# UbiquityRobotics/fiducials

Measured on AMD Instinct MI355X. Metric: frames/sec @1920x1080 20-marker (aruco detect + pose hot path), higher is better.
Workload: dtype u8

## Files before the change

fiducials_amd/csrc/fid_api.hip:

```cpp
#include "fid_kernels.hip"

#include <math.h>
#include <stdio.h>
#include <stdlib.h>
#include <string.h>

#include <new>
#include <string>
#include <vector>

namespace {

enum { ST_GRAY = 0, ST_THRESH, ST_STARTS, ST_PROBE, ST_WALK, ST_APPROX, ST_SORT, ST_NEAR, ST_RESOLVE, ST_IDENT, ST_FILTER, ST_SUBPIX, ST_POSE, ST_SEEDWALK,
       ST_SEEDLESS, ST_COUNT };
const char *const kStageNames[ST_COUNT] = {"to_gray", "threshold", "find_starts", "walk_probe", "walk_full", "approx", "sort_cands",
                                           "near", "resolve", "identify", "filter_markers", "subpix", "pose", "seed_walk", "seedless_chain"};

constexpr int TX = 128, TY = 32, NT = 256;
constexpr int THRW_NT = 512, THRW_WT = 16;
static_assert(THRW_NT * THRW_WT >= 8191, "k_threshold_wide: a row per workgroup");

}

struct fid_ctx {
    int device = 0;
    hipStream_t stream = nullptr;
    enum { MAX_SUB = 8 };
    hipStream_t sub_stream[MAX_SUB] = {};
    int sub_prio[MAX_SUB] = {};
    hipStream_t aux_stream[MAX_SUB] = {};
    hipStream_t idx_stream = nullptr;
    hipEvent_t aux_fork[MAX_SUB] = {}, aux_join[MAX_SUB] = {}, aux_idx[MAX_SUB] = {};
    hipEvent_t sub_done[MAX_SUB] = {}, fork_ev = nullptr;
    hipStream_t copy_stream = nullptr;
    hipEvent_t in_ready[MAX_SUB] = {};
    bool host_feed = false;
    struct Pending {
        const uint8_t *d_src;
        int F, W, H, stride;
        long long fstride;
        fid_encoding enc;
    } pend = {};
    bool in_flight = false;
    hipEvent_t tail_ev = nullptr, wait_ev = nullptr;
    hipEvent_t wait_copy_ev = nullptr;
    bool fed_from_host = false;
    int chain_at = 0;
    bool chained = false;
    hipEvent_t walk_done[MAX_SUB] = {}, fs_done[MAX_SUB] = {}, front_done[MAX_SUB] = {};
    int pieces = 0;
    bool piece_chain = false;
    bool from_host_call = false;
    int fs_barrier = 0;
    int stagger = 0;
    int resolve_lds_kb = 64;
    int walk2_div = 6;
    int probe_refill0 = 0;
    int probe_refill = 4;
    hipEvent_t sub_ev[MAX_SUB][20] = {};
    int sub_frames = 0;
    fid_params params;
    fid_limits lim;
    DevParams P;
    std::vector<uint8_t> dict_host;
    int dict_ms = 0, dict_maxc = 0, dict_n = 0;
    uint8_t *d_in = nullptr;
    size_t d_in_bytes = 0;
    uint8_t *d_gray = nullptr;
    uint32_t *d_masks = nullptr;
    size_t masks_bytes = 0;
    int masks_W = 0, masks_H = 0, masks_S = 0;
    uint2 *d_starts = nullptr, *d_surv1 = nullptr, *d_surv = nullptr;
    uint32_t *d_pool = nullptr;
    DevSegC *d_segs = nullptr;
    DevPend *d_pend = nullptr;
    uint2 *d_seedq = nullptr;
    unsigned long long *d_seedhash = nullptr;
    int seed_hash_cap = 0, seed_gen = 0;
    uint4 *d_wres = nullptr, *d_cinfo = nullptr;
    uint32_t *d_cbase = nullptr, *d_dense = nullptr;
    uint4 *d_recs = nullptr;
    int thr_xcd = 1;
    int thr_nw = 3, thr_split = 0, thr_rows = 0;
    bool whole_border_walk = false;
    int sw_blocks = 0;
    int tail_grid = 4096;
    int filter_lds = 256;
    int light_x = 1;
    long long fallbacks = 0;
    int max_chunks = 0;
    int walk_blocks = 0;
    int walk_blocks_cap = 0;
    int copy_blocks = 0;
    int resolve_serial = 0;
    int resolve_reg_max = 64;
    int seed_shift = 0;
    uint4 *d_contours = nullptr;
    uint32_t *d_ckpts = nullptr;
    size_t ckpts_elems = 0;
    DevCand *d_cands = nullptr, *d_sorted = nullptr, *d_filtered = nullptr;
    float4 *d_cmeta = nullptr;
    uint32_t *d_near = nullptr;
    DevIdent *d_ident = nullptr;
    uint8_t *d_bits = nullptr;
    int bits_cap = 0;
    fid_marker *d_pre = nullptr, *d_markers = nullptr, *d_filter_scratch = nullptr;
    int *d_accsrc = nullptr, *d_mksrc = nullptr;
    fid_pose_out *d_poses = nullptr;
    DevCounts *d_counts = nullptr;
    DevGlobal *d_global = nullptr;
    unsigned *d_worklist = nullptr, *d_nwork = nullptr;
    uint8_t *d_dict = nullptr;
    float *d_subpix_mask = nullptr;
    uint8_t *d_probe_tables = nullptr;
    double *d_lens = nullptr;
    fid_marker *d_pose_in = nullptr;
    int *d_pose_n = nullptr;
    int pose_cap = 0;
    uint8_t *d_res = nullptr, *h_res = nullptr;
    size_t res_clear_bytes = 0, res_markers_end = 0, res_poses_end = 0, res_poses_off = 0;
    bool blocking = false;
    bool res_precleared = false;
    fid_marker *h_markers = nullptr;
    DevCounts *h_counts = nullptr;
    DevGlobal *h_global = nullptr;
    fid_pose_out *h_poses = nullptr;
    bool pose_cam_valid = false, pose_done = false;
    fid_camera pose_cam = {};
    double pose_len = 0.;
    int *d_map_ids = nullptr;
    double *d_map_obj = nullptr;
    int map_n = 0;
    fid_map_pose_out *d_mposes = nullptr, *h_mposes = nullptr;
    fid_marker *d_map_in = nullptr;
    int map_in_cap = 0;
    bool map_cam_valid = false, map_done = false;
    fid_camera map_cam = {};
    int last_frames = 0, last_W = 0, last_H = 0, last_nsub = 1;
    const uint8_t *last_gray = nullptr;
    long long last_gfstride = 0;
    bool profile = false;
    hipEvent_t ev[ST_COUNT + 1] = {};
    bool ev_valid[ST_COUNT + 1] = {};
    float stage_ms[ST_COUNT] = {};
    std::string last_error;
};

static void map_pose_launch(fid_ctx *c, hipStream_t st, const fid_marker *d_markers, const int *d_n, int n_stride_ints, int per_frame, int F,
                            const fid_camera &camera, fid_map_pose_out *d_out);

namespace {

#define HIPCHK(ctx, expr)                                                                         \
    do {                                                                                          \
        hipError_t e_ = (expr);                                                                   \
        if (e_ != hipSuccess) {                                                                   \
            (ctx)->last_error = std::string(#expr) + ": " + hipGetErrorString(e_);                \
            return e_ == hipErrorOutOfMemory ? FID_E_OUT_OF_MEMORY : FID_E_HIP;                   \
        }                                                                                         \
    } while (0)

template <typename T>
fid_status dalloc(fid_ctx *c, T **p, size_t count)
{
    HIPCHK(c, hipMalloc((void **)p, count * sizeof(T)));
    return FID_OK;
}

int roundup(int v, int m) { return (v + m - 1) / m * m; }

size_t results_bytes(int F, int MM)
{
    auto up = [](size_t v) { return (v + 255) & ~(size_t)255; };
    return up(sizeof(DevGlobal)) + up(sizeof(unsigned) * fid_ctx::MAX_SUB) + up(sizeof(DevCounts) * (size_t)F) + up(sizeof(fid_marker) * (size_t)F * MM) +
           up(sizeof(fid_pose_out) * (size_t)F * MM);
}
void layout_results(fid_ctx *c, int F)
{
    auto up = [](size_t v) { return (v + 255) & ~(size_t)255; };
// ... 306 lines not shown
        const fid_status rcs = ensure_streams(c, nsub, F);
        if (rcs != FID_OK) return rcs;
    }
    if (nsub > 1) HIPCHK(c, hipEventRecord(c->fork_ev, st0));
    bool tail_recorded = false;
    auto sub_phase = [&](int sb, int phase) -> fid_status {
        const int f0 = plan.f0[sb], Fs = plan.f0[sb + 1] - f0;
        hipStream_t st = nsub > 1 ? c->sub_stream[chainp ? (sb & 1) : sb] : st0;
        if (nsub > 1 && phase == 0) HIPCHK(c, hipStreamWaitEvent(st, c->fork_ev, 0));
        if (chainp && phase == 0 && sb > 0) HIPCHK(c, hipStreamWaitEvent(st, c->fs_done[sb - 1], 0));
        if (c->host_feed && phase == 0) HIPCHK(c, hipStreamWaitEvent(st, c->in_ready[sb], 0));
        if (nsub > 1 && phase == 0 && c->stagger > 0 && sb >= c->stagger) HIPCHK(c, hipStreamWaitEvent(st, c->walk_done[sb - c->stagger], 0));
        DevParams P = c->P;
        P.nframes = Fs;
        const size_t MC = (size_t)P.maxCands, MM = (size_t)P.maxMarkers;
        const uint8_t *g = gray + (long long)f0 * gfstride;
        uint32_t *masks = c->d_masks + (size_t)f0 * P.nscales * P.TR * P.TC * MT_ROWS;
        uint2 *starts = c->d_starts + (size_t)f0 * P.maxStarts, *surv1 = c->d_surv1 + (size_t)f0 * P.maxStarts,
              *surv = c->d_surv + (size_t)f0 * P.maxStarts;
        uint4 *contours = c->d_contours + (size_t)f0 * P.maxContours;
        uint32_t *tab = c->d_ckpts + (size_t)f0 * 2 * P.maxContours * chunk_tab_pitch(P);
        uint32_t *pool = c->d_pool + (size_t)f0 * P.maxChunks * CKW;
        DevCounts *counts = c->d_counts + f0;
        DevCand *cands = c->d_cands + f0 * MC, *sorted = c->d_sorted + f0 * MC, *filtered = c->d_filtered + f0 * MC;
        uint32_t *nearb = c->d_near + f0 * MC * (MC / 32);
        DevIdent *ident = c->d_ident + f0 * MC;
        fid_marker *pre = c->d_pre + f0 * MM, *markers = c->d_markers + f0 * MM;
        unsigned *worklist = c->d_worklist + f0 * MC, *nwork = c->d_nwork + sb;
        hipEvent_t *ev = c->sub_ev[sb];
        auto mark = [&](int idx) {
            if (c->profile) (void)hipEventRecord(ev[idx], st);
        };
        auto chain_point = [&](int pt) {
            if (sb == nsub - 1 && !tail_recorded && !c->blocking && c->chain_at <= pt) {
                (void)hipEventRecord(c->tail_ev, st);
                tail_recorded = true;
            }
        };
      if (phase == 0) {
        mark(0);
        if (to_gray && (int)enc <= FID_ENC_RGBA8)
            hipLaunchKernelGGL(k_to_gray, dim3(2048), dim3(256), 0, st, d_src + (long long)f0 * fstride, stride, fstride, (int)enc,
                               c->d_gray + (size_t)f0 * W * H, W, H, Fs);
        else if (to_gray)
            hipLaunchKernelGGL(k_raw_to_gray, dim3((W + 255) / 256, (H + 3) / 4, Fs), dim3(64, 4), 0, st, d_src + (long long)f0 * fstride, stride,
                               fstride, (int)enc, c->d_gray + (size_t)f0 * W * H, W, H);
        mark(ST_GRAY + 1);
        {
            bool node_table = P.nscales == 13;
            for (int i = 0; i < P.nscales && node_table; i++) node_table = P.win[i] == 3 + 4 * i;
            if (node_table) {
                const int cols = 64 * c->thr_nw, strips = (W + cols - 1) / cols;
                int RS = c->thr_rows;
                if (RS <= 0) {
                    int segs = (1536 + strips * Fs - 1) / (strips * Fs);
                    const int maxsegs = (H + 63) / 64;
                    segs = segs < 1 ? 1 : (segs > maxsegs ? maxsegs : segs);
                    RS = (H + segs - 1) / segs;
                }
                RS = (RS + 3) & ~3;
                dim3 grid(strips, (H + RS - 1) / RS, Fs);
                if (c->thr_nw == 5 && c->thr_split) launch_thr_stream<5, true>(grid, st, g, gfstride, masks, P, RS, c->thr_xcd);
                else if (c->thr_nw == 5) launch_thr_stream<5, false>(grid, st, g, gfstride, masks, P, RS, c->thr_xcd);
                else if (c->thr_split) launch_thr_stream<3, true>(grid, st, g, gfstride, masks, P, RS, c->thr_xcd);
                else launch_thr_stream<3, false>(grid, st, g, gfstride, masks, P, RS, c->thr_xcd);
            } else if (P.rmax > 40) {
                int bands = (512 + Fs - 1) / Fs;
                const int maxb = (H + 15) / 16;
                bands = bands < 1 ? 1 : (bands > maxb ? maxb : bands);
                const int BH = (H + bands - 1) / bands;
                const size_t lds = (size_t)(W + 1 + THRW_NT / 64) * sizeof(unsigned long long);
                fid_launch_log("k_threshold_wide", THRW_NT, lds);
                hipLaunchKernelGGL((k_threshold_wide<THRW_NT, THRW_WT>), dim3((H + BH - 1) / BH, 1, Fs), dim3(THRW_NT), lds, st, g, gfstride,
                                   masks, P, BH);
            } else {
                int R = P.rmax, RW = TX + 2 * R, RH = TY + 2 * R, PT = (RW + 1) | 1;
                size_t lds = (size_t)(RH + 1) * PT * sizeof(uint32_t);
                dim3 grid((W + TX - 1) / TX, (H + TY - 1) / TY, Fs);
                hipLaunchKernelGGL((k_threshold<TX, TY, NT>), grid, dim3(NT), lds, st, g, gfstride, masks, P);
            }
        }
        mark(ST_THRESH + 1);
      }
        long long k2blocks;
        {
            long long groups = (long long)P.nscales * P.TR * ((P.WW + 15) / 16);
            k2blocks = (groups + 7) / 8;
            if (k2blocks > 256) k2blocks = 256;
        }
      if (phase == 0) {
        if (!c->whole_border_walk) {
            hipLaunchKernelGGL(k_find_starts<true>, dim3((unsigned)k2blocks, Fs), dim3(256), 0, st, masks, starts, counts, c->d_global,
                               c->d_seedq + f0 * (size_t)P.maxContours, P);
            mark(ST_STARTS + 1);
            if (nsub > 1) HIPCHK(c, hipEventRecord(c->fs_done[sb], st));
            chain_point(0);
        }
        return FID_OK;
      }
        if (!c->whole_border_walk && nsub > 1 && c->fs_barrier && !chainp)
            for (int o = 0; o < nsub; o++)
                if (o != sb) HIPCHK(c, hipStreamWaitEvent(st, c->fs_done[o], 0));
        int wb = c->walk_blocks > 0 ? c->walk_blocks : (3072 / WALK_WAVES + Fs - 1) / Fs;
        const int wcap = c->walk_blocks_cap > 0 ? c->walk_blocks_cap : (Fs <= 2 ? 256 : 64);
        wb = wb < 2 ? 2 : (wb > wcap ? wcap : wb);
        const int gm = Fs >= 16 ? 1 : 16 / Fs;
        const int wb2 = wb > 1 ? wb / 2 : 1;
        const int cap1 = pts_cap_first(P);
        const size_t lds1 = k_approx_lds_bytes(cap1);
        const size_t lds2 = k_approx_lds_bytes(P.maxPerim + 1);
        if (c->whole_border_walk) {
            hipLaunchKernelGGL(k_find_starts<false>, dim3((unsigned)k2blocks, Fs), dim3(256), 0, st, masks, starts, counts, c->d_global,
                               (uint2 *)nullptr, P);
            mark(ST_STARTS + 1);
            hipLaunchKernelGGL((k_probe<PROBE0_STEPS, 0>), dim3(64 * gm, Fs), dim3(256), 0, st, masks, starts, surv1, counts, c->d_global, P);
            hipLaunchKernelGGL((k_probe<PROBE1_STEPS, 1>), dim3(16 * gm, Fs), dim3(256), 0, st, masks, surv1, surv, counts, c->d_global, P);
            mark(ST_PROBE + 1);
            hipLaunchKernelGGL(k_walk_full<0>, dim3(wb, Fs), dim3(64 * WALK_WAVES), 0, st, masks, surv, contours, tab, pool, (DevSegC *)nullptr,
                               (DevPend *)nullptr, counts, c->d_global, P);
            mark(ST_WALK + 1);
            fid_launch_log("k_approx", 64, (size_t)(lds1));
            hipLaunchKernelGGL(k_approx, dim3(128 * gm, Fs), dim3(64), lds1, st, contours, tab, pool, cands, counts, P, cap1, 0,
                               (const uint32_t *)nullptr, (const uint32_t *)nullptr);
            fid_launch_log("k_approx", 64, (size_t)(lds2));
            hipLaunchKernelGGL(k_approx, dim3(16 * gm, Fs), dim3(64), lds2, st, contours, tab, pool, cands, counts, P,
                               P.maxPerim + 1, 1, (const uint32_t *)nullptr, (const uint32_t *)nullptr);
            mark(ST_APPROX + 1);
        } else {
            const size_t MCn = (size_t)P.maxContours;
            DevSegC *segs = c->d_segs + f0 * MCn;
            DevPend *pend = c->d_pend + f0 * MCn;
            uint2 *seedq = c->d_seedq + f0 * MCn;
            unsigned long long *seedhash = c->d_seedhash + (size_t)f0 * P.seedHashCap;
            uint4 *wres = c->d_wres + f0 * MCn, *cinfo = c->d_cinfo + f0 * MCn;
            uint32_t *cbase = c->d_cbase + f0 * MCn;
            uint32_t *dense = c->d_dense + (size_t)f0 * P.maxChunks * (CK / 4);
            hipStream_t sa = c->aux_stream[chainp ? (sb & 1) : sb];
            HIPCHK(c, hipEventRecord(c->aux_fork[sb], st));
            HIPCHK(c, hipStreamWaitEvent(sa, c->aux_fork[sb], 0));
            int swb = c->sw_blocks > 0 ? c->sw_blocks : (1024 / SW_WAVES + Fs - 1) / Fs;
            swb = swb < 2 ? 2 : (swb > 4 * wcap ? 4 * wcap : swb);
            uint4 *recs = c->d_recs + 2 * f0 * MCn;
            const int cpb = c->copy_blocks > 0 ? c->copy_blocks : 256;
            if (c->profile) (void)hipEventRecord(ev[14], st);
            hipLaunchKernelGGL(k_seed_walk, dim3(swb, Fs), dim3(64 * SW_WAVES), 0, st, masks, seedq, tab, pool, segs, counts, c->d_global, P);
            if (c->profile) (void)hipEventRecord(ev[15], st);
            mark(ST_PROBE + 1);
            chain_point(1);
            if (c->profile) (void)hipEventRecord(ev[16], sa);
            hipStream_t si = (nsub == 1 && Fs <= 16 && c->idx_stream) ? c->idx_stream : sa;
            if (si != sa) HIPCHK(c, hipStreamWaitEvent(si, c->aux_fork[sb], 0));
            hipLaunchKernelGGL(k_seed_index, dim3(8 * gm, Fs), dim3(256), 0, si, seedq, seedhash, counts, P);
            HIPCHK(c, hipEventRecord(c->aux_idx[sb], si));
            if (c->probe_refill0 && gm == 1)
                hipLaunchKernelGGL((k_probe_refill<PROBE0_STEPS, 0>), dim3(c->probe_refill0, Fs), dim3(256), 0, sa, masks, starts, surv1, counts, c->d_global, P,
                                   (const uint4 *)c->d_probe_tables);
            else
                hipLaunchKernelGGL((k_probe_lut<PROBE0_STEPS, 0>), dim3(64 * gm, Fs), dim3(256), 0, sa, masks, starts, surv1, counts, c->d_global, P,
                                   (const uint4 *)c->d_probe_tables);
            if (c->probe_refill && gm == 1)
                hipLaunchKernelGGL((k_probe_refill<PROBE1_STEPS, 1>), dim3(c->probe_refill, Fs), dim3(256), 0, sa, masks, surv1, surv, counts, c->d_global, P,
                                   (const uint4 *)c->d_probe_tables);
            else
                hipLaunchKernelGGL((k_probe_lut<PROBE1_STEPS, 1>), dim3(16 * gm, Fs), dim3(256), 0, sa, masks, surv1, surv, counts, c->d_global, P,
                                   (const uint4 *)c->d_probe_tables);
            const int wb3 = c->walk2_div > 0 ? (wb / c->walk2_div > 0 ? wb / c->walk2_div : 1) : wb2;
            hipLaunchKernelGGL(k_walk_full<2>, dim3(wb3, Fs), dim3(64 * WALK_WAVES), 0, sa, masks, surv, wres, tab, pool, segs, pend, counts,
                               c->d_global, P);
            if (si != sa) HIPCHK(c, hipStreamWaitEvent(sa, c->aux_idx[sb], 0));
            hipLaunchKernelGGL(k_seg_cycles<0>, dim3(8 * gm, Fs), dim3(64), 0, sa, seedq, segs, pend, wres, contours, cinfo, cbase,
                               recs, counts, c->d_global, P, 1, 0);
            hipLaunchKernelGGL(k_seg_copy, dim3(cpb / 4 > 0 ? cpb / 4 : 1, Fs), dim3(256), 0, sa, recs, tab, pool, dense, counts, P, 1);
            fid_launch_log("k_approx", 64, (size_t)(lds1));
            hipLaunchKernelGGL(k_approx, dim3(32 * gm, Fs), dim3(64), lds1, sa, contours, tab, pool, cands, counts, P, cap1, 0,
                               dense, cbase, 2);
            fid_launch_log("k_approx", 64, (size_t)(lds2));
            hipLaunchKernelGGL(k_approx, dim3(8 * gm, Fs), dim3(64), lds2, sa, contours, tab, pool, cands, counts, P,
// ... 250 lines not shown
    memset(p, 0, sizeof(*p));
    p->adaptiveThreshConstant = 7;
    p->adaptiveThreshWinSizeMin = 3;
    p->adaptiveThreshWinSizeMax = 53;
    p->adaptiveThreshWinSizeStep = 4;
    p->cornerRefinementMethod = 1;
    p->cornerRefinementWinSize = 5;
    p->cornerRefinementMaxIterations = 30;
    p->cornerRefinementMinAccuracy = 0.01;
    p->errorCorrectionRate = 0.6;
    p->minCornerDistanceRate = 0.05;
    p->markerBorderBits = 1;
    p->minDistanceToBorder = 3;
    p->maxErroneousBitsInBorderRate = 0.04;
    p->minMarkerDistanceRate = 0.05;
    p->minMarkerPerimeterRate = 0.1;
    p->maxMarkerPerimeterRate = 4.0;
    p->minOtsuStdDev = 5.0;
    p->perspectiveRemoveIgnoredMarginPerCell = 0.13;
    p->perspectiveRemovePixelPerCell = 8;
    p->polygonalApproxAccuracyRate = 0.01;
}

void fid_default_limits(fid_limits *l)
{
    if (!l) return;
    memset(l, 0, sizeof(*l));
    l->max_width = 1920;
    l->max_height = 1080;
    l->max_batch = 1;
    l->max_starts_per_frame = 262144;
    l->max_contours_per_frame = 16384;
    l->max_candidates_per_frame = 2048;
    l->max_markers_per_frame = 256;
    l->max_points_per_frame = 4 * 1024 * 1024;
}

fid_status fid_create(const fid_params *params, const fid_dict *dict, const fid_limits *limits, int device, fid_ctx **out)
{
    if (!params || !dict || !out || !dict->bytes || dict->n_markers <= 0 || dict->marker_size < 3 || dict->marker_size > 7)
        return FID_E_INVALID_ARG;
    *out = nullptr;
    int ndev = 0;
    if (hipGetDeviceCount(&ndev) != hipSuccess || ndev <= 0) return FID_E_NO_DEVICE;
    if (device < 0 || device >= ndev) return FID_E_INVALID_ARG;
    fid_ctx *c = new (std::nothrow) fid_ctx();
    if (!c) return FID_E_OUT_OF_MEMORY;
    c->device = device;
    fid_limits L;
    fid_default_limits(&L);
    if (limits) {
        if (limits->max_width > 0) L.max_width = limits->max_width;
        if (limits->max_height > 0) L.max_height = limits->max_height;
        if (limits->max_batch > 0) L.max_batch = limits->max_batch;
        if (limits->max_starts_per_frame > 0) L.max_starts_per_frame = limits->max_starts_per_frame;
        if (limits->max_contours_per_frame > 0) L.max_contours_per_frame = limits->max_contours_per_frame;
        if (limits->max_candidates_per_frame > 0) L.max_candidates_per_frame = limits->max_candidates_per_frame;
        if (limits->max_markers_per_frame > 0) L.max_markers_per_frame = limits->max_markers_per_frame;
        if (limits->max_points_per_frame > 0) L.max_points_per_frame = limits->max_points_per_frame;
    }
    if (L.max_batch <= 4) {
        if (!limits || limits->max_contours_per_frame <= 0) L.max_contours_per_frame = 65536;
        if (!limits || limits->max_points_per_frame <= 0) L.max_points_per_frame = 16 * 1024 * 1024;
    } else if (L.max_batch <= 16) {
        if (!limits || limits->max_contours_per_frame <= 0) L.max_contours_per_frame = 32768;
        if (!limits || limits->max_points_per_frame <= 0) L.max_points_per_frame = 8 * 1024 * 1024;
    }
    L.max_candidates_per_frame = roundup(L.max_candidates_per_frame, 32);
    if (L.max_candidates_per_frame > 4096 || L.max_batch > 65535 || L.max_markers_per_frame > L.max_candidates_per_frame ||
        L.max_contours_per_frame > (1 << 20)) {
        delete c;
        return FID_E_INVALID_ARG;
    }
    c->lim = L;
    c->dict_ms = dict->marker_size;
    c->dict_maxc = dict->max_correction_bits;
    c->dict_n = dict->n_markers;
    size_t dbytes = (size_t)dict->n_markers * 4 * ((dict->marker_size * dict->marker_size + 7) / 8);
    c->dict_host.assign(dict->bytes, dict->bytes + dbytes);
    c->profile = getenv("FID_PROFILE") && atoi(getenv("FID_PROFILE")) != 0;
    if (getenv("FID_SUB_FRAMES")) c->sub_frames = atoi(getenv("FID_SUB_FRAMES"));
    if (getenv("FID_WALK_CAP")) c->walk_blocks_cap = atoi(getenv("FID_WALK_CAP"));
    if (getenv("FID_SEED_SHIFT")) c->seed_shift = atoi(getenv("FID_SEED_SHIFT"));
    if (getenv("FID_RESOLVE_SERIAL")) c->resolve_serial = atoi(getenv("FID_RESOLVE_SERIAL"));
    if (getenv("FID_RESOLVE_REG_MAX")) {
        const int v = atoi(getenv("FID_RESOLVE_REG_MAX"));
        c->resolve_reg_max = v < 0 ? 0 : (v > 64 ? 64 : v);
    }
    if (getenv("FID_COPY_BLOCKS")) c->copy_blocks = atoi(getenv("FID_COPY_BLOCKS"));
    if (getenv("FID_THR_NW")) c->thr_nw = atoi(getenv("FID_THR_NW")) == 3 ? 3 : 5;
    if (getenv("FID_THR_SPLIT")) c->thr_split = atoi(getenv("FID_THR_SPLIT")) != 0;
    if (getenv("FID_THR_ROWS")) c->thr_rows = atoi(getenv("FID_THR_ROWS"));
    if (getenv("FID_THR_XCD")) c->thr_xcd = atoi(getenv("FID_THR_XCD")) != 0;
    if (getenv("FID_WALK_BLOCKS")) c->walk_blocks = atoi(getenv("FID_WALK_BLOCKS")) > 0 ? atoi(getenv("FID_WALK_BLOCKS")) : c->walk_blocks;
    memset(&c->P, 0, sizeof(c->P));

    fid_status rc = FID_OK;
    auto fail = [&](fid_status s) {
        fid_destroy(c);
        return s;
    };
#define TRY(expr)                         \
    do {                                  \
        rc = (expr);                      \
        if (rc != FID_OK) return fail(rc); \
    } while (0)
#define TRYHIP(expr)                                   \
    do {                                               \
        hipError_t e_ = (expr);                        \
        if (e_ != hipSuccess) {                        \
            fprintf(stderr, "fid_create: %s: %s\n", #expr, hipGetErrorString(e_)); \
            return fail(e_ == hipErrorOutOfMemory ? FID_E_OUT_OF_MEMORY : FID_E_HIP); \
        }                                              \
    } while (0)
    TRYHIP(hipSetDevice(device));
    TRYHIP(hipStreamCreateWithFlags(&c->stream, hipStreamNonBlocking));
    for (int i = 0; i <= ST_COUNT; i++) TRYHIP(hipEventCreate(&c->ev[i]));
    TRYHIP(hipEventCreateWithFlags(&c->fork_ev, hipEventDisableTiming));
    TRYHIP(hipEventCreateWithFlags(&c->tail_ev, hipEventDisableTiming));
    int prio_lo = 0, prio_hi = 0;
    (void)hipDeviceGetStreamPriorityRange(&prio_lo, &prio_hi);
    const bool use_prio = getenv("FID_PRIO") && atoi(getenv("FID_PRIO"));
    for (int sb = 0; sb < fid_ctx::MAX_SUB; sb++) {
        int prio = use_prio ? prio_hi + sb : prio_lo;
        if (prio > prio_lo) prio = prio_lo;
        c->sub_prio[sb] = prio;
        TRYHIP(hipEventCreateWithFlags(&c->aux_fork[sb], hipEventDisableTiming));
        TRYHIP(hipEventCreateWithFlags(&c->aux_join[sb], hipEventDisableTiming));
        TRYHIP(hipEventCreateWithFlags(&c->sub_done[sb], hipEventDisableTiming));
        TRYHIP(hipEventCreateWithFlags(&c->walk_done[sb], hipEventDisableTiming));
        TRYHIP(hipEventCreateWithFlags(&c->in_ready[sb], hipEventDisableTiming));
        TRYHIP(hipEventCreateWithFlags(&c->fs_done[sb], hipEventDisableTiming));
        TRYHIP(hipEventCreateWithFlags(&c->front_done[sb], hipEventDisableTiming));
        TRYHIP(hipEventCreateWithFlags(&c->aux_idx[sb], hipEventDisableTiming));
        for (int i = 0; i < 20; i++) TRYHIP(hipEventCreate(&c->sub_ev[sb][i]));
    }
    const size_t F = L.max_batch, MC = L.max_candidates_per_frame, MM = L.max_markers_per_frame;
    TRY(dalloc(c, &c->d_subpix_mask, (size_t)(2 * SP_MAXWIN_MAX + 1) * (2 * SP_MAXWIN_MAX + 1)));
    TRY(dalloc(c, &c->d_probe_tables, (size_t)4096));
    hipLaunchKernelGGL(k_probe_tables, dim3(1), dim3(256), 0, nullptr, c->d_probe_tables);
    TRYHIP(hipGetLastError());
    TRYHIP(hipDeviceSynchronize());
    TRY(dalloc(c, &c->d_dict, dbytes));
    TRYHIP(hipMemcpy(c->d_dict, c->dict_host.data(), dbytes, hipMemcpyHostToDevice));
    rc = apply_params(c, params);
    if (rc != FID_OK) return fail(rc);
    TRY(dalloc(c, &c->d_gray, F * L.max_width * L.max_height));
    c->masks_bytes = masks_elems(c, L.max_width, L.max_height, (int)F) * sizeof(uint32_t);
    c->masks_bytes += (size_t)F * c->P.nscales * (L.max_height + 2) * 16 * sizeof(uint32_t);
    TRYHIP(hipMalloc((void **)&c->d_masks, c->masks_bytes));
    TRY(dalloc(c, &c->d_starts, F * L.max_starts_per_frame));
    TRY(dalloc(c, &c->d_surv1, F * L.max_starts_per_frame));
    TRY(dalloc(c, &c->d_surv, F * L.max_starts_per_frame));
    c->max_chunks = (L.max_points_per_frame + CK - 1) / CK;
    TRY(dalloc(c, &c->d_pool, F * (size_t)c->max_chunks * CKW));
    c->whole_border_walk = getenv("FID_TRACE") && !strcmp(getenv("FID_TRACE"), "legacy");
    if (getenv("FID_SW_BLOCKS")) c->sw_blocks = atoi(getenv("FID_SW_BLOCKS"));
    if (getenv("FID_STAGGER")) c->stagger = atoi(getenv("FID_STAGGER"));
    if (getenv("FID_PIECES")) c->pieces = atoi(getenv("FID_PIECES"));
    if (getenv("FID_FS_BARRIER")) c->fs_barrier = atoi(getenv("FID_FS_BARRIER"));
    if (getenv("FID_TAIL_GRID")) c->tail_grid = atoi(getenv("FID_TAIL_GRID"));
    if (getenv("FID_FILTER_LDS")) c->filter_lds = atoi(getenv("FID_FILTER_LDS")) > 0 ? atoi(getenv("FID_FILTER_LDS")) : 1;
    if (getenv("FID_LIGHT_X")) c->light_x = atoi(getenv("FID_LIGHT_X")) > 0 ? atoi(getenv("FID_LIGHT_X")) : 1;
    if (getenv("FID_RESOLVE_LDS")) c->resolve_lds_kb = atoi(getenv("FID_RESOLVE_LDS"));
    if (getenv("FID_WALK2_DIV")) c->walk2_div = atoi(getenv("FID_WALK2_DIV"));
    if (getenv("FID_PROBE_REFILL")) c->probe_refill = atoi(getenv("FID_PROBE_REFILL"));
// ... 712 lines not shown
```

fiducials_amd/csrc/fid_kernels.hip:

```cpp
#include <hip/hip_runtime.h>
#include <stdint.h>
#include <float.h>
#include <limits.h>

#include <type_traits>
#include <utility>

#include "fid_device.h"
#include "../../include/fid_abi.h"

#define WAVE 64

__device__ __forceinline__ int lane_id() { return threadIdx.x & (WAVE - 1); }

__device__ __forceinline__ unsigned long long ballot64(int pred) { return __ballot(pred); }

#define FID_DPP(OLD, V, CTRL, RMASK) __builtin_amdgcn_update_dpp((OLD), (V), (CTRL), (RMASK), 0xf, false)
#define FID_DPP_SCAN_STEPS(STEP) STEP(0x111, 0xf) STEP(0x112, 0xf) STEP(0x114, 0xf) STEP(0x118, 0xf) STEP(0x142, 0xa) STEP(0x143, 0xc)

__device__ __forceinline__ int wave_iscan(int v)
{
#define S_(C, M) v += FID_DPP(0, v, C, M);
    FID_DPP_SCAN_STEPS(S_)
#undef S_
// ... 963 lines not shown
        if (lane == 63) {
            s_wsum[0][wid] = incl;
            s_wsum[1][wid] = sincl;
        }
        __syncthreads();
        int wbase = 0, tot = 0, swbase = 0, stot = 0;
#pragma unroll
        for (int k = 0; k < 4; k++) {
            const int v = s_wsum[0][k], sv2 = s_wsum[1][k];
            if (k < wid) {
                wbase += v;
                swbase += sv2;
            }
            tot += v;
            stot += sv2;
        }
        if (threadIdx.x == 0) {
#ifdef FS_NOATOMIC
            if (tot) s_base[0] = (unsigned)(blockIdx.x * 977u + (unsigned)i0) % (cap - 64u);
            if (HYB && stot) s_base[1] = (unsigned)(blockIdx.x * 331u + (unsigned)i0) % (scap - 64u);
#else
            if (tot) s_base[0] = atomicAdd((unsigned *)&counts[f].nstarts, (unsigned)tot);
            if (HYB && stot) s_base[1] = atomicAdd((unsigned *)&counts[f].nseeds, (unsigned)stot);
#endif
        }
        __syncthreads();
        if (tot) {
            unsigned off = s_base[0] + (unsigned)(wbase + incl - cnt);
#pragma unroll
            for (int r = 0; r < 2; r++) {
                if (!cntv[r]) continue;
                const uint32_t meta = (uint32_t)f | ((uint32_t)sv[r] << 16);
#pragma unroll
                for (int k = 0; k < 4; k++) {
                    const uint32_t y = (uint32_t)(yy0v[r] + k - 1);
                    uint32_t o = outer[r][k], hh = hole[r][k];
                    while (o) {
                        int b = __ffs(o) - 1;
                        o &= o - 1;
                        if (off < cap) fst[off] = make_uint2((uint32_t)(x_base[r] + b) | (y << 16), meta);
                        off++;
                    }
                    while (hh) {
                        int b = __ffs(hh) - 1;
                        hh &= hh - 1;
                        if (off < cap) fst[off] = make_uint2((uint32_t)(x_base[r] + b) | (y << 16), meta | (1u << 24));
                        off++;
                    }
                }
            }
            if (threadIdx.x == 0 && s_base[0] + (unsigned)tot > cap) atomicOr(&G->overflow, 1u);
        }
        if (HYB && stot) {
            unsigned off = s_base[1] + (unsigned)(swbase + sincl - scnt);
            auto emit = [&](int x, int y, int sc, int dd) {
                if (off < scap) fsq[off] = make_uint2((uint32_t)x | ((uint32_t)y << 13) | ((uint32_t)sc << 27), (uint32_t)dd);
                off++;
            };
#pragma unroll
            for (int r = 0; r < 2; r++) {
                if (!scntv[r]) continue;
                {
                    const int y = yy0v[r] + rowk[r] - 1;
                    int ri = 0;
#pragma unroll
                    for (int dd = 0; dd < 8; dd++) {
                        if (!((SEED_DIRS_ROW >> dd) & 1u)) continue;
                        uint32_t m = rowm[r][ri++];
                        while (m) {
                            const int b = __ffs(m) - 1;
                            m &= m - 1;
                            emit(x_base[r] + b, y, sv[r], dd);
                        }
                    }
                }
                uint32_t cb = colb[r];
                while (cb) {
                    const int b = __ffs(cb) - 1;
                    cb &= cb - 1;
                    emit(x_base[r], yy0v[r] + (b >> 3) - 1, sv[r], b & 7);
                }
            }
            if (threadIdx.x == 0 && s_base[1] + (unsigned)stot > scap) atomicOr(&G->overflow, 2u);
        }
        __syncthreads();
    }
}


__device__ __forceinline__ int dir_dx(int d) { return (int)((0x901Au >> (2 * d)) & 3u) - 1; }
__device__ __forceinline__ int dir_dy(int d) { return (int)((0xA901u >> (2 * d)) & 3u) - 1; }

struct MaskView {
    const uint32_t *base;
    int TC;
};

__device__ __forceinline__ unsigned nb8(const MaskView &m, int x, int y)
{
    const int xb = x - 1 + MASK_PADW * 32;
    const int wi = xb >> 5, sh = xb & 31;
    const bool two = sh > 29;
    const uint32_t *p0 = m.base + mask_word(m.TC, y, wi);
    const uint32_t *p1 = m.base + mask_word(m.TC, y + 1, wi);
    const uint32_t *p2 = m.base + mask_word(m.TC, y + 2, wi);
    const uint32_t a0 = p0[0], a1 = p1[0], a2 = p2[0];
    uint32_t b0 = 0, b1 = 0, b2 = 0;
    if (two) {
        b0 = p0[MT_ROWS];
        b1 = p1[MT_ROWS];
        b2 = p2[MT_ROWS];
    }
    unsigned tu = __builtin_amdgcn_alignbit(b0, a0, sh) & 7u;
    unsigned tm = __builtin_amdgcn_alignbit(b1, a1, sh) & 7u;
    unsigned td = __builtin_amdgcn_alignbit(b2, a2, sh) & 7u;
    return ((tm >> 2) & 1u) | (((tu >> 2) & 1u) << 1) | (((tu >> 1) & 1u) << 2) | ((tu & 1u) << 3) | ((tm & 1u) << 4) |
           ((td & 1u) << 5) | (((td >> 1) & 1u) << 6) | (((td >> 2) & 1u) << 7);
}

__device__ __forceinline__ int pidx(int x, int y, int W) { return (y + 1) * (W + 2) + (x + 1); }

#define CK 64
#define CKW 8
#define REC_NO_CHUNK 0xffffffffu
__device__ __forceinline__ uint32_t code_delta(unsigned c)
{
    const unsigned c2 = (c & 7u) * 2u;
    return (((0x901Au >> c2) & 3u) | (((0xA901u >> c2) & 3u) << 16)) - 0x10001u;
}
__device__ __forceinline__ uint2 codes_nibbles_to_bytes(uint32_t w)
{
    uint32_t a = w & 0xffffu, b = w >> 16;
    a = (a | (a << 8)) & 0x00ff00ffu;
    b = (b | (b << 8)) & 0x00ff00ffu;
    return make_uint2((a | (a << 4)) & 0x0f0f0f0fu, (b | (b << 4)) & 0x0f0f0f0fu);
}
__device__ __forceinline__ uint32_t codes8_to_points(uint32_t *pts, int k, int count, uint32_t base, uint2 w)
{
    uint32_t p[8], s = 0;
    const uint32_t w2[2] = {w.x << 1, w.y << 1};
#pragma unroll
    for (int i = 0; i < 8; i++) {
        const unsigned c2 = (w2[i >> 2] >> (8 * (i & 3))) & 14u;
        p[i] = s - (uint32_t)i * 0x10001u;
        s += ((0x901Au >> c2) & 3u) | (((0xA901u >> c2) & 3u) << 16);
    }
    s -= 8u * 0x10001u;
    const uint32_t incl = wave_iscan_dpp(s);
    const uint32_t mine = base + incl - s;
    if (k < count) {
        *reinterpret_cast<uint4 *>(pts + k) = make_uint4(mine + p[0], mine + p[1], mine + p[2], mine + p[3]);
        *reinterpret_cast<uint4 *>(pts + k + 4) = make_uint4(mine + p[4], mine + p[5], mine + p[6], mine + p[7]);
    }
    return base + (uint32_t)__builtin_amdgcn_readlane((int)incl, 63);
}
__device__ __host__ inline int chunk_tab_pitch(const DevParams &P) { return P.maxPerim / CK + 3; }
__device__ __forceinline__ long long chunk_tab_at(const DevParams &P, int f, unsigned row, unsigned k)
{
    return ((long long)f * chunk_tab_pitch(P) + k) * (2ll * P.maxContours) + row;
}

#ifndef PROBE0_STEPS
#define PROBE0_STEPS 6
#endif
#ifndef PROBE1_STEPS
#define PROBE1_STEPS 32
// ... 3404 lines not shown
```

Measured before the change: 40170.

## Split seed discovery out of find_starts into a dedicated seed kernel

Adds a standalone k_find_seeds kernel that scans row and column seed units independently and writes the seed queue. When seedShift is at least 4, or when forced by an environment variable, find_starts runs without seed emission and the new kernel runs after it. The aim is to parallelize seed discovery better than the fused path. The cost is an extra launch and a second pass over the masks.

```diff
diff --git a/fiducials_amd/csrc/fid_api.hip b/fiducials_amd/csrc/fid_api.hip
--- a/fiducials_amd/csrc/fid_api.hip
+++ b/fiducials_amd/csrc/fid_api.hip
@@ -95,6 +95,7 @@
     int resolve_serial = 0;
     int resolve_reg_max = 64;
     int seed_shift = 0;
+    int seed_kernel = 0;
     uint4 *d_contours = nullptr;
     uint32_t *d_ckpts = nullptr;
     size_t ckpts_elems = 0;
@@ -567,6 +568,7 @@
         }
         mark(ST_THRESH + 1);
       }
+        const bool split_seeds = c->seed_kernel ? c->seed_kernel == 1 : P.seedShift >= 4;
         long long k2blocks;
         {
             long long groups = (long long)P.nscales * P.TR * ((P.WW + 15) / 16);
@@ -575,9 +577,18 @@
         }
       if (phase == 0) {
         if (!c->whole_border_walk) {
-            hipLaunchKernelGGL(k_find_starts<true>, dim3((unsigned)k2blocks, Fs), dim3(256), 0, st, masks, starts, counts, c->d_global,
-                               c->d_seedq + f0 * (size_t)P.maxContours, P);
-            mark(ST_STARTS + 1);
+            uint2 *seedq = c->d_seedq + f0 * (size_t)P.maxContours;
+            if (split_seeds) {
+                const SeedUnits su = seed_units(P);
+                const int smax = Fs >= 16 ? 32 : 512, sblocks = (su.n + 3) / 4 < smax ? (su.n + 3) / 4 : smax;
+                hipLaunchKernelGGL(k_find_starts<false>, dim3((unsigned)k2blocks, Fs), dim3(256), 0, st, masks, starts, counts, c->d_global,
+                                   (uint2 *)nullptr, P);
+                mark(ST_STARTS + 1);
+                hipLaunchKernelGGL(k_find_seeds, dim3(sblocks, Fs), dim3(256), 0, st, masks, counts, c->d_global, seedq, P);
+            } else {
+                hipLaunchKernelGGL(k_find_starts<true>, dim3((unsigned)k2blocks, Fs), dim3(256), 0, st, masks, starts, counts, c->d_global, seedq, P);
+                mark(ST_STARTS + 1);
+            }
             if (nsub > 1) HIPCHK(c, hipEventRecord(c->fs_done[sb], st));
             chain_point(0);
         }
@@ -994,6 +1005,7 @@
     if (getenv("FID_SUB_FRAMES")) c->sub_frames = atoi(getenv("FID_SUB_FRAMES"));
     if (getenv("FID_WALK_CAP")) c->walk_blocks_cap = atoi(getenv("FID_WALK_CAP"));
     if (getenv("FID_SEED_SHIFT")) c->seed_shift = atoi(getenv("FID_SEED_SHIFT"));
+    if (const char *e = getenv("FID_SEED_KERNEL")) c->seed_kernel = !strcmp(e, "split") ? 1 : (!strcmp(e, "fused") ? 2 : 0);
     if (getenv("FID_RESOLVE_SERIAL")) c->resolve_serial = atoi(getenv("FID_RESOLVE_SERIAL"));
     if (getenv("FID_RESOLVE_REG_MAX")) {
         const int v = atoi(getenv("FID_RESOLVE_REG_MAX"));
diff --git a/fiducials_amd/csrc/fid_kernels.hip b/fiducials_amd/csrc/fid_kernels.hip
--- a/fiducials_amd/csrc/fid_kernels.hip
+++ b/fiducials_amd/csrc/fid_kernels.hip
@@ -1069,6 +1069,161 @@
                 }
             }
             if (threadIdx.x == 0 && s_base[1] + (unsigned)stot > scap) atomicOr(&G->overflow, 2u);
+        }
+        __syncthreads();
+    }
+}
+
+struct SeedUnits {
+    int nrows, ncols, nwc, nqc, nquads, urow, n;
+};
+__host__ __device__ inline SeedUnits seed_units(const DevParams &P)
+{
+    SeedUnits u;
+    const int gm = (8 << P.seedShift) - 1, wsh = P.seedShift - 2;
+    u.nrows = (P.H + gm) >> (P.seedShift + 3);
+    u.ncols = (P.WW + (1 << wsh) - 1) >> wsh;
+    u.nquads = P.H / 4 + 1;
+    u.nwc = (P.WW + 63) >> 6;
+    u.nqc = (u.nquads + 63) >> 6;
+    u.urow = P.nscales * u.nrows * u.nwc;
+    u.n = u.urow + P.nscales * u.ncols * u.nqc;
+    return u;
+}
+__global__ __launch_bounds__(256) void k_find_seeds(const uint32_t *__restrict__ masks, DevCounts *__restrict__ counts,
+                                                     DevGlobal *__restrict__ G, uint2 *__restrict__ seedq, const DevParams P)
+{
+    __shared__ int s_wsum[4];
+    __shared__ unsigned s_base;
+    const int lane = lane_id(), wid = __builtin_amdgcn_readfirstlane(threadIdx.x >> 6);
+    const int f = blockIdx.y;
+    const int WW = P.WW, TC = P.TC, H = P.H;
+    const SeedUnits U = seed_units(P);
+    const float rcp_nwc = 1.0f / (float)U.nwc, rcp_nqc = 1.0f / (float)U.nqc, rcp_nrows = 1.0f / (float)U.nrows, rcp_ncols = 1.0f / (float)U.ncols;
+    const long long plane = (long long)P.TR * TC * MT_ROWS;
+    const unsigned scap = (unsigned)P.maxContours;
+    const int gm = (8 << P.seedShift) - 1;
+    const uint32_t *fmasks = masks + (long long)f * P.nscales * plane;
+    uint2 *fsq = seedq + (long long)f * P.maxContours;
+    for (int i0 = (int)blockIdx.x * 4; i0 < U.n; i0 += (int)gridDim.x * 4) {
+        const int unit = i0 + wid;
+        uint32_t rowm[6] = {0, 0, 0, 0, 0, 0}, colb = 0;
+        int cnt = 0, x0 = 0, y0 = 0, sc = 0;
+        const bool is_row = unit < U.urow;
+        if (is_row) {
+            unsigned a, wc, s, j;
+            divmod_small((unsigned)unit, (unsigned)U.nwc, rcp_nwc, a, wc);
+            divmod_small(a, (unsigned)U.nrows, rcp_nrows, s, j);
+            sc = __builtin_amdgcn_readfirstlane((int)s);
+            y0 = __builtin_amdgcn_readfirstlane((int)j) << (P.seedShift + 3);
+            const int w = __builtin_amdgcn_readfirstlane((int)wc) * 64 + lane;
+            x0 = w * 32;
+            if (w < WW) {
+                const uint32_t *tile = fmasks + (long long)sc * plane + ((long long)(y0 >> 4) * TC + MASK_PADW + w) * MT_ROWS;
+                const uint4 c4 = *reinterpret_cast<const uint4 *>(tile);
+                const uint32_t cur = c4.y;
+                if (cur) {
+                    const uint4 p4 = *reinterpret_cast<const uint4 *>(tile - MT_ROWS);
+                    const uint4 n4 = *reinterpret_cast<const uint4 *>(tile + MT_ROWS);
+                    const uint32_t u = c4.x, d = c4.z;
+                    const uint32_t Wst = (cur << 1) | (p4.y >> 31), Est = (cur >> 1) | (n4.y << 31);
+                    const uint32_t NW = (u << 1) | (p4.x >> 31), NE = (u >> 1) | (n4.x << 31);
+                    const uint32_t SWst = (d << 1) | (p4.z >> 31), SEst = (d >> 1) | (n4.z << 31);
+                    const uint32_t nbp[8] = {Est, NE, u, NW, Wst, SWst, d, SEst};
+                    int ri = 0;
+#pragma unroll
+                    for (int dd = 0; dd < 8; dd++) {
+                        if (!((SEED_DIRS_ROW >> dd) & 1u)) continue;
+                        const uint32_t m = cur & nbp[dd] & ~nbp[seed_empty_dir(dd)];
+                        rowm[ri++] = m;
+                        cnt += __popc(m);
+                    }
+                }
+            }
+        } else if (unit < U.n) {
+            unsigned a, qc, s, ci;
+            divmod_small((unsigned)(unit - U.urow), (unsigned)U.nqc, rcp_nqc, a, qc);
+            divmod_small(a, (unsigned)U.ncols, rcp_ncols, s, ci);
+            sc = __builtin_amdgcn_readfirstlane((int)s);
+            const int w = __builtin_amdgcn_readfirstlane((int)ci) << (P.seedShift - 2);
+            const int q = __builtin_amdgcn_readfirstlane((int)qc) * 64 + lane;
+            x0 = w * 32;
+            y0 = q * 4;
+            if (q < U.nquads) {
+                const uint32_t *pl = fmasks + (long long)sc * plane;
+                const uint32_t *tile = pl + mask_word(TC, y0, MASK_PADW + w);
+                const uint4 c4 = *reinterpret_cast<const uint4 *>(tile);
+                if ((c4.x | c4.y | c4.z | c4.w) & 1u) {
+                    const uint4 p4 = *reinterpret_cast<const uint4 *>(tile - MT_ROWS);
+                    uint32_t upc = 0, upp = 0;
+                    if (y0 > 0) {
+                        const uint32_t *qq = pl + mask_word(TC, y0 - 1, MASK_PADW + w);
+                        upc = qq[0];
+                        upp = qq[-MT_ROWS];
+                    }
+                    const uint32_t *qq = pl + mask_word(TC, y0 + 4, MASK_PADW + w);
+                    const uint32_t cc[6] = {upc, c4.x, c4.y, c4.z, c4.w, qq[0]};
+                    const uint32_t pp[6] = {upp, p4.x, p4.y, p4.z, p4.w, qq[-MT_ROWS]};
+#pragma unroll
+                    for (int k = 0; k < 4; k++) {
+                        const int y = y0 + k - 1;
+                        if (y < 0 || y >= H) continue;
+                        const uint32_t cur = cc[k + 1], u = cc[k], d = cc[k + 2];
+                        uint32_t n8 = (cur >> 1) & 1u;
+                        n8 |= u & 2u;
+                        n8 |= (u & 1u) << 2;
+                        n8 |= (pp[k] >> 31) << 3;
+                        n8 |= (pp[k + 1] >> 31) << 4;
+                        n8 |= (pp[k + 2] >> 31) << 5;
+                        n8 |= (d & 3u) << 6;
+                        const uint32_t x16 = n8 | (n8 << 8);
+                        const uint32_t e8 = ((x16 >> 1) & 0xAAu) | ((x16 >> 2) & 0x55u);
+                        const uint32_t allowed = (y & gm) == 0 ? (SEED_DIRS_COL & ~SEED_DIRS_ROW) : SEED_DIRS_COL;
+                        const uint32_t s8 = (cur & 1u) ? (n8 & ~e8 & allowed) : 0u;
+                        colb |= s8 << (k * 8);
+                    }
+                    cnt = __popc(colb);
+                }
+            }
+        }
+        const int incl = wave_iscan(cnt);
+        if (lane == 63) s_wsum[wid] = incl;
+        __syncthreads();
+        int wbase = 0, tot = 0;
+#pragma unroll
+        for (int k = 0; k < 4; k++) {
+            const int v = s_wsum[k];
+            if (k < wid) wbase += v;
+            tot += v;
+        }
+        if (threadIdx.x == 0 && tot) s_base = atomicAdd((unsigned *)&counts[f].nseeds, (unsigned)tot);
+        __syncthreads();
+        if (tot) {
+            unsigned off = s_base + (unsigned)(wbase + incl - cnt);
+            auto emit = [&](int x, int y, int dd) {
+                if (off < scap) fsq[off] = make_uint2((uint32_t)x | ((uint32_t)y << 13) | ((uint32_t)sc << 27), (uint32_t)dd);
+                off++;
+            };
+            if (is_row) {
+                int ri = 0;
+#pragma unroll
+                for (int dd = 0; dd < 8; dd++) {
+                    if (!((SEED_DIRS_ROW >> dd) & 1u)) continue;
+                    uint32_t m = rowm[ri++];
+                    while (m) {
+                        const int b = __ffs(m) - 1;
+                        m &= m - 1;
+                        emit(x0 + b, y0, dd);
+                    }
+                }
+            } else {
+                while (colb) {
+                    const int b = __ffs(colb) - 1;
+                    colb &= colb - 1;
+                    emit(x0, y0 + (b >> 3) - 1, b & 7);
+                }
+            }
+            if (threadIdx.x == 0 && s_base + (unsigned)tot > scap) atomicOr(&G->overflow, 2u);
         }
         __syncthreads();
     }
```

After: 40900, median of 6. 1.8% higher.
